# linnil1/KIR_graph

Hardware: AMD Instinct MI355X
Metric: typed 150 bp PE reads/s (pileup+EM) per GPU; achieved HBM GB/s vs roofline (higher is better)
Workload: dtype f64

## Files before the change

include/graphkir_hip.h:

```cpp
#ifndef GRAPHKIR_HIP_H
#define GRAPHKIR_HIP_H

#include <stddef.h>
#include <stdint.h>

#ifdef __cplusplus
extern "C" {
#endif

#define GK_ABI_VERSION 1

#define GK_OK 0
#define GK_ERR_NO_DEVICE (-1)
#define GK_ERR_HIP (-2)
#define GK_ERR_ARG (-3)
#define GK_ERR_ASSERT (-4)
#define GK_ERR_CAPACITY (-5)

#define GK_MAX_CIG 14
#define GK_MAX_MM 16
#define GK_MAX_INS 6
#define GK_MAX_EVENTS 22
#define GK_CIG_M 0
#define GK_CIG_I 1
// ... 132 lines not shown
                       int32_t n_entries, int32_t n_slots, uint64_t* totals_out, int64_t max_out, int32_t* slot_out,
                       int32_t* ord_out, uint32_t* count_out, uint64_t* key_out, int64_t* n_out);

int gk_lut_create(gk_ctx* ctx, int32_t log2_capacity, gk_lut** out);
int gk_lut_destroy(gk_lut* lut);
int gk_lut_collect(gk_lut* lut, gk_dptr d_vals, int64_t n);
int gk_lut_pending(gk_lut* lut, int32_t* n_total, int32_t* n_known);
int gk_lut_export(gk_lut* lut, int32_t first, int32_t count, double* keys_out);
int gk_lut_define(gk_lut* lut, int32_t first, int32_t count, const double* log_vals);
int gk_lut_apply(gk_lut* lut, gk_dptr d_in, gk_dptr d_out, int64_t n);
typedef int (*gk_log10_fn)(const double* values, int64_t n, double* out);
int gk_lut_resolve(gk_lut* lut, gk_log10_fn log10_fn, int32_t* n_new, int32_t* n_known, int32_t* n_undefined);
int gk_lut_resolve_stored(gk_lut* lut, gk_log10_fn log10_fn, int32_t* n_new, int32_t* n_known, int32_t* n_undefined);
int gk_lut_known(gk_lut* lut, int32_t* n_known);
int gk_compat_log(gk_ctx* ctx, gk_tab* tab, gk_dptr d_rows, int64_t n_rows, gk_dptr d_vflag,
                  int32_t vbeg, int32_t vend, gk_dptr d_mask, int32_t words, int32_t n_allele, int32_t keep_empty,
                  gk_lut* lut, gk_dptr d_log);

int gk_maxsum(gk_ctx* ctx, gk_dptr d_L, int64_t n_rows, int64_t ld, const int32_t* ids, int32_t n_sets,
              int32_t c_prev, const int32_t* cols, int32_t n_cols, double* out);
int gk_fraction(gk_ctx* ctx, gk_dptr d_L, int64_t n_rows, int64_t ld, const int32_t* ids,
                int32_t n_sets, int32_t c, double* frac_out);
int gk_setmax(gk_ctx* ctx, gk_dptr d_L, int64_t n_rows, int64_t ld, const int32_t* ids, int32_t n_sets,
              int32_t c, gk_dptr d_P);

int gk_compat_log_miss(gk_ctx* ctx, gk_tab* tab, gk_dptr d_rows, int64_t n_rows, gk_dptr d_vflag,
                       int32_t vbeg, int32_t vend, gk_dptr d_mask, int32_t words, int32_t n_allele,
                       int32_t keep_empty, gk_lut* lut, gk_dptr d_log, gk_dptr d_miss8, int64_t ldm, gk_dptr d_flags);
int gk_miss_colsum(gk_ctx* ctx, gk_dptr d_miss8, int64_t ldm, int32_t n_cols, gk_dptr d_msum);
int gk_compat_log_miss_cols(gk_ctx* ctx, gk_tab* tab, gk_dptr d_rows, int64_t n_rows, gk_dptr d_vflag,
                            int32_t vbeg, int32_t vend, gk_dptr d_mask, int32_t words, int32_t n_allele,
                            int32_t keep_empty, gk_lut* lut, const int32_t* table_cols, int32_t n_table_cols,
                            gk_dptr d_log, gk_dptr d_miss8, int64_t ldm, gk_dptr d_flags);
int gk_compat_patch(gk_ctx* ctx, gk_lut* lut, gk_dptr d_log, int64_t n_rows, int32_t n_allele, gk_dptr d_miss8,
                    int64_t ldm, gk_dptr d_flags);
int gk_compat_index(gk_ctx* ctx, gk_tab* tab, gk_dptr d_rows, int64_t n_rows, gk_dptr d_vflag, int32_t vbeg,
                    int32_t vend, gk_dptr d_mask, int32_t words, int32_t n_allele, int32_t keep_empty, gk_lut* lut,
                    gk_dptr d_lidx, gk_dptr d_miss8, int64_t ldm, gk_dptr d_flags);
int gk_expand_index(gk_ctx* ctx, gk_lut* lut, gk_dptr d_lidx, int64_t ldi, int64_t n_rows, int32_t n_allele, gk_dptr d_L,
                    int64_t ld);
int gk_bound_step(gk_ctx* ctx, gk_dptr d_miss8, int64_t ldm, int64_t n_rows, gk_dptr d_msum, const int32_t* ids,
                  int32_t n_sets, int32_t c_prev, const int32_t* cols, int32_t n_cols, const uint8_t* first,
                  int32_t top_n, int32_t cap, uint32_t* hdr_out, int32_t* idx_out, uint32_t* m_out);
int gk_setsum(gk_ctx* ctx, gk_dptr d_L, int64_t n_rows, int64_t ld, const int32_t* ids, int32_t n_sets, int32_t c,
              double* value_out, double* frac_out);

typedef int (*gk_argsort_fn)(const double* values, int64_t n, int64_t* order_out);
typedef struct gk_search gk_search;
int gk_search_run(gk_ctx* ctx, gk_dptr d_L, int64_t n_rows, int64_t ld, int32_t n_allele, gk_dptr d_miss8,
                  int64_t ldm, gk_dptr d_msum, const int32_t* cols, int32_t n_cols, int32_t n_steps, int32_t top_n,
                  gk_argsort_fn argsort, const double* colsum_in, gk_search** out);
typedef struct gk_gene_job {
  gk_dptr d_rows;
  int64_t n_rows;
  gk_dptr d_mask;
  gk_dptr d_L;
  gk_dptr d_miss8;
  int64_t ldm;
  gk_dptr d_msum;
  gk_dptr d_flags;
  gk_dptr d_lidx;
  int32_t vbeg, vend;
  int32_t words, n_allele;
  int32_t n_steps, top_n;
  int32_t bound_ok, passes;
  int32_t indexed, patches;
// ... 128 lines not shown
```

kir_graph_amd/_lib.py:

```python
from __future__ import annotations

import ctypes as C
import threading
import os
from pathlib import Path

import numpy as np

LIB_NAME = "libgraphkir_hip.so"
_lib = None


class GkError(RuntimeError):
    """Error reported by the native library."""


class GkNoDevice(GkError):
    """No HIP device: the typing path cannot run (there is no CPU fallback)."""


_MM = np.dtype([("ref_off", "<u2"), ("base", "u1"), ("rsv", "u1")])
MATE_DTYPE = np.dtype([
    ("pos0", "<u4"), ("flag", "<u2"), ("ref", "u1"), ("nh", "u1"),
    ("nm", "u1"), ("n_cig", "u1"), ("n_mm", "u1"), ("n_ins", "u1"),
# ... 136 lines not shown
    "gk_bam_next": (C.c_int, [C.c_void_p, C.c_void_p, C.c_int64, C.POINTER(C.c_int64)]),
    "gk_compat_log": (C.c_int, [C.c_void_p, C.c_void_p, C.c_uint64, C.c_int64, C.c_uint64, C.c_int32, C.c_int32,
                                C.c_uint64, C.c_int32, C.c_int32, C.c_int32, C.c_void_p, C.c_uint64]),
    "gk_maxsum": (C.c_int, [C.c_void_p, C.c_uint64, C.c_int64, C.c_int64, C.c_void_p, C.c_int32, C.c_int32,
                            C.c_void_p, C.c_int32, C.c_void_p]),
    "gk_fraction": (C.c_int, [C.c_void_p, C.c_uint64, C.c_int64, C.c_int64, C.c_void_p, C.c_int32, C.c_int32,
                              C.c_void_p]),
    "gk_setmax": (C.c_int, [C.c_void_p, C.c_uint64, C.c_int64, C.c_int64, C.c_void_p, C.c_int32, C.c_int32,
                            C.c_uint64]),
    "gk_packer_create": (C.c_int, [C.c_void_p, C.c_int32, C.c_void_p, C.c_int32, C.POINTER(C.c_void_p)]),
    "gk_packer_destroy": (C.c_int, [C.c_void_p]),
    "gk_packer_feed": (C.c_int, [C.c_void_p, C.c_char_p, C.c_size_t, C.c_int32]),
    "gk_packer_counts": (C.c_int, [C.c_void_p, C.POINTER(C.c_int64), C.POINTER(C.c_int64), C.POINTER(C.c_int64),
                                   C.POINTER(C.c_int64), C.POINTER(C.c_int64)]),
    "gk_packer_error": (C.c_int, [C.c_void_p, C.POINTER(C.c_int32), C.POINTER(C.c_int64)]),
    "gk_packer_records": (C.c_int, [C.c_void_p, C.c_void_p, C.c_void_p]),
    "gk_packer_set_output": (C.c_int, [C.c_void_p, C.c_void_p, C.c_int64]),
    "gk_packer_spilled": (C.c_int, [C.c_void_p, C.POINTER(C.c_int64)]),
    "gk_packer_spill_records": (C.c_int, [C.c_void_p, C.c_void_p, C.c_void_p]),
    "gk_packer_string": (C.c_char_p, [C.c_void_p, C.c_int64]),
    "gk_depth": (C.c_int, [C.c_void_p, C.c_void_p, C.c_uint64, C.c_int32, C.c_void_p, C.c_int32, C.c_void_p]),
    "gk_depth_write_tsv": (C.c_int, [C.c_char_p, C.c_void_p, C.c_void_p, C.c_int32, C.c_void_p]),
    "gk_cn_fit": (C.c_int, [C.c_void_p, C.c_void_p, C.c_void_p, C.c_int32, C.c_void_p, C.c_int32, C.c_void_p,
                            C.c_int32, C.c_int32, C.c_double, C.c_void_p]),
    "gk_cn_assign": (C.c_int, [C.c_void_p, C.c_void_p, C.c_int32, C.c_double, C.c_void_p, C.c_int32, C.c_int32,
                               C.c_double, C.c_void_p]),
    "gk_em_sets": (C.c_int, [C.c_void_p, C.c_void_p, C.c_uint64, C.c_int64, C.c_int32, C.c_int32, C.c_uint64,
                             C.c_int32, C.c_uint64]),
    "gk_em_distinct": (C.c_int, [C.c_void_p, C.c_uint64, C.c_int64, C.c_int32, C.c_int32, C.c_void_p, C.c_void_p,
                                 C.POINTER(C.c_int32)]),
    "gk_compat_log_miss_cols": (C.c_int, [C.c_void_p, C.c_void_p, C.c_uint64, C.c_int64, C.c_uint64, C.c_int32, C.c_int32,
                                          C.c_uint64, C.c_int32, C.c_int32, C.c_int32, C.c_void_p, C.c_void_p, C.c_int32,
                                          C.c_uint64, C.c_uint64, C.c_int64, C.c_uint64]),
    "gk_compat_log_miss": (C.c_int, [C.c_void_p, C.c_void_p, C.c_uint64, C.c_int64, C.c_uint64, C.c_int32, C.c_int32,
                                     C.c_uint64, C.c_int32, C.c_int32, C.c_int32, C.c_void_p, C.c_uint64, C.c_uint64,
                                     C.c_int64, C.c_uint64]),
    "gk_miss_colsum": (C.c_int, [C.c_void_p, C.c_uint64, C.c_int64, C.c_int32, C.c_uint64]),
    "gk_compat_index": (C.c_int, [C.c_void_p, C.c_void_p, C.c_uint64, C.c_int64, C.c_uint64, C.c_int32, C.c_int32,
                                  C.c_uint64, C.c_int32, C.c_int32, C.c_int32, C.c_void_p, C.c_uint64, C.c_uint64,
                                  C.c_int64, C.c_uint64]),
    "gk_expand_index": (C.c_int, [C.c_void_p, C.c_void_p, C.c_uint64, C.c_int64, C.c_int64, C.c_int32, C.c_uint64,
                                  C.c_int64]),
    "gk_bound_step": (C.c_int, [C.c_void_p, C.c_uint64, C.c_int64, C.c_int64, C.c_uint64, C.c_void_p, C.c_int32,
                                C.c_int32, C.c_void_p, C.c_int32, C.c_void_p, C.c_int32, C.c_int32, C.c_void_p,
                                C.c_void_p, C.c_void_p]),
    "gk_setsum": (C.c_int, [C.c_void_p, C.c_uint64, C.c_int64, C.c_int64, C.c_void_p, C.c_int32, C.c_int32,
                            C.c_void_p, C.c_void_p]),
    "gk_search_run": (C.c_int, [C.c_void_p, C.c_uint64, C.c_int64, C.c_int64, C.c_int32, C.c_uint64, C.c_int64,
                                C.c_uint64, C.c_void_p, C.c_int32, C.c_int32, C.c_int32, C.c_void_p, C.c_void_p,
                                C.POINTER(C.c_void_p)]),
    "gk_sample_search": (C.c_int, [C.c_void_p, C.c_void_p, C.c_int32, C.c_void_p, C.c_uint64, C.c_void_p, C.c_void_p,
                                   C.c_int32, C.c_void_p, C.c_void_p, C.c_void_p]),
    "gk_lut_resolve": (C.c_int, [C.c_void_p, C.c_void_p, C.POINTER(C.c_int32), C.POINTER(C.c_int32),
                                 C.POINTER(C.c_int32)]),
    "gk_sample_prepare_exon": (C.c_int, [C.c_void_p, C.c_void_p, C.c_int32, C.c_uint64, C.c_uint64, C.c_uint64, C.c_void_p,
                                         C.c_int64, C.c_void_p, C.c_void_p, C.c_void_p, C.POINTER(C.c_int64)]),
    "gk_sample_em": (C.c_int, [C.c_void_p, C.c_void_p, C.c_void_p, C.c_int32, C.c_int32, C.c_double, C.c_void_p, C.c_void_p]),
    "gk_mates_compact": (C.c_int, [C.c_void_p, C.c_uint64, C.c_int64, C.POINTER(C.c_uint64), C.POINTER(C.c_int64)]),
    "gk_mates_expand": (C.c_int, [C.c_void_p, C.c_uint64, C.c_int64, C.c_uint64]),
    "gk_mates_compact_size": (C.c_int, [C.c_void_p, C.c_int64, C.c_int32, C.POINTER(C.c_int64)]),
    "gk_mates_compact_host": (C.c_int, [C.c_void_p, C.c_int64, C.c_int32, C.c_void_p, C.c_int64]),
    "gk_compat_patch": (C.c_int, [C.c_void_p, C.c_void_p, C.c_uint64, C.c_int64, C.c_int32, C.c_uint64, C.c_int64, C.c_uint64]),
    "gk_lut_resolve_stored": (C.c_int, [C.c_void_p, C.c_void_p, C.POINTER(C.c_int32), C.POINTER(C.c_int32),
                                        C.POINTER(C.c_int32)]),
    "gk_lut_known": (C.c_int, [C.c_void_p, C.POINTER(C.c_int32)]),
    "gk_search_steps": (C.c_int, [C.c_void_p, C.POINTER(C.c_int32)]),
# ... 288 lines not shown
```

kir_graph_amd/build.py:

```python
from __future__ import annotations

import os
import shutil
import subprocess
from pathlib import Path

PKG = Path(__file__).resolve().parent
ROOT = PKG.parent
SOURCES = ["gk_runtime.hip", "gk_scan.hip", "gk_tabulate.hip", "gk_typing.hip", "gk_lut.hip",
           "gk_search.hip", "gk_bound.hip", "gk_em.hip", "gk_cn.hip", "gk_depth.hip", "gk_sampack.cpp", "gk_bamread.cpp", "gk_textout.cpp",
           "gk_comm.cpp", "gk_hostsearch.cpp", "gk_novel.hip", "gk_boot.hip"]


def hipcc() -> str:
    for cand in (os.environ.get("HIPCC"), shutil.which("hipcc"), "/opt/rocm/bin/hipcc"):
        if cand and Path(cand).exists():
            return cand
    raise RuntimeError("hipcc not found (set HIPCC)")


def outOfDate(lib: Path) -> bool:
    if not lib.exists():
        return True
    t = lib.stat().st_mtime
    deps = [PKG / "csrc" / s for s in SOURCES] + list((PKG / "csrc").glob("*.h")) + [ROOT / "include" / "graphkir_hip.h"]
    return any(d.stat().st_mtime > t for d in deps)


KERNEL_SOURCES = {
    "compat_kernel": ["gk_typing.hip", "gk_lut.h", "gk_common.h"],
    "patch_pending": ["gk_typing.hip", "gk_lut.h", "gk_common.h"],
    "count_ids_genes": ["gk_typing.hip", "gk_common.h"],
    "flag_nonempty": ["gk_typing.hip", "gk_common.h"],
    "flag_pairs": ["gk_typing.hip", "gk_common.h"],
    "gather_pair_flags": ["gk_typing.hip", "gk_common.h"],
    "tab_count": ["gk_tabulate.hip", "gk_common.h"],
    "tab_emit": ["gk_tabulate.hip", "gk_common.h"],
    "tab_expand": ["gk_tabulate.hip", "gk_common.h"],
    "minsum_sad": ["gk_bound.hip", "gk_common.h"],
    "minsum_finish": ["gk_bound.hip", "gk_common.h"],
    "select_hist1": ["gk_bound.hip", "gk_common.h"],
    "select_hist2": ["gk_bound.hip", "gk_common.h"],
    "select_append": ["gk_bound.hip", "gk_common.h"],
    "setmin_u8": ["gk_bound.hip", "gk_common.h"],
    "fraction_chunks": ["gk_search.hip", "gk_common.h"],
    "setsum_leaves": ["gk_search.hip", "gk_common.h"],
    "fold_leaves": ["gk_search.hip", "gk_common.h"],
    "colsum_chunks": ["gk_search.hip", "gk_common.h"],
    "maxsum_chunks": ["gk_search.hip", "gk_common.h"],
    "combine_chunks": ["gk_search.hip", "gk_common.h"],
    "em_sets_groups": ["gk_em.hip", "gk_common.h"],
    "em_sets_hash": ["gk_em.hip", "gk_common.h"],
    "em_sets_verify": ["gk_em.hip", "gk_common.h"],
    "em_sets_emit": ["gk_em.hip", "gk_common.h"],
    "em_kernel_genes": ["gk_em.hip", "gk_squarem.h", "gk_common.h"],
    "novel_assign": ["gk_novel.hip", "gk_common.h"],
    "novel_confusion": ["gk_novel.hip", "gk_common.h"],
    "novel_compact": ["gk_novel.hip", "gk_common.h"],
    "boot_resample": ["gk_boot.hip", "gk_common.h"],
    "boot_em_batch": ["gk_boot.hip", "gk_squarem.h", "gk_common.h"],
}


# ... 51 lines not shown
```

kir_graph_amd/csrc/gk_hostsearch.cpp:

```cpp
#include <algorithm>
#include <cmath>
#include <memory>
#include <numeric>
#include <string>
#include <unordered_map>
#include <unordered_set>
#include <chrono>
#include <sys/syscall.h>
#include <unistd.h>

#include "gk_calls.h"
#include "gk_lut.h"

namespace {

struct Step {
  int n = 0;
  int bounded = 0;
  std::vector<double> value, sum_indv, frac;
  std::vector<int32_t> ids;
  int64_t rows() const { return (int64_t)value.size(); }
};

inline double sum_small(const double* a, int n) {
// ... 139 lines not shown
    for (size_t i = 0; i < n; ++i)
      if (!seen[ids[i]]) { seen[ids[i]] = 1; ++d; }
    return d;
  }
  void note(int64_t kind, int64_t a, int64_t b, int64_t c, int64_t d, int64_t e, int64_t f) {
    const int64_t row[7] = {kind, a, b, c, d, e, f};
    log.insert(log.end(), row, row + 7);
  }
  void to_alleles(const int32_t* cols, int n_cols, int n_alleles) {
    for (Step& st : steps)
      for (int32_t& id : st.ids) id = cols[id];
    table_cols.assign(cols, cols + n_cols);
    n_full = n_alleles;
  }
};

extern "C" {

int gk_maxsum(gk_ctx* ctx, gk_dptr d_L, int64_t n_rows, int64_t ld, const int32_t* ids, int32_t n_sets, int32_t c_prev,
              const int32_t* cols, int32_t n_cols, double* out);
int gk_fraction(gk_ctx* ctx, gk_dptr d_L, int64_t n_rows, int64_t ld, const int32_t* ids, int32_t n_sets, int32_t c,
                double* frac_out);
int gk_compat_log_miss(gk_ctx* ctx, gk_tab* tab, gk_dptr d_rows, int64_t n_rows, gk_dptr d_vflag, int32_t vbeg,
                       int32_t vend, gk_dptr d_mask, int32_t words, int32_t n_allele, int32_t keep_empty, gk_lut* lut,
                       gk_dptr d_log, gk_dptr d_miss8, int64_t ldm, gk_dptr d_flags);
int gk_compat_log(gk_ctx* ctx, gk_tab* tab, gk_dptr d_rows, int64_t n_rows, gk_dptr d_vflag, int32_t vbeg,
                  int32_t vend, gk_dptr d_mask, int32_t words, int32_t n_allele, int32_t keep_empty, gk_lut* lut,
                  gk_dptr d_log);
__attribute__((weak)) int gk_compat_log_miss_cols(gk_ctx* ctx, gk_tab* tab, gk_dptr d_rows, int64_t n_rows, gk_dptr d_vflag,
                                                  int32_t vbeg, int32_t vend, gk_dptr d_mask, int32_t words, int32_t n_allele,
                                                  int32_t keep_empty, gk_lut* lut, const int32_t* table_cols,
                                                  int32_t n_table_cols, gk_dptr d_log, gk_dptr d_miss8, int64_t ldm,
                                                  gk_dptr d_flags);
int gk_miss_colsum(gk_ctx* ctx, gk_dptr d_miss8, int64_t ldm, int32_t n_cols, gk_dptr d_msum);
int gk_compat_patch(gk_ctx* ctx, gk_lut* lut, gk_dptr d_log, int64_t n_rows, int32_t n_allele, gk_dptr d_miss8, int64_t ldm,
                    gk_dptr d_flags);
int gk_compat_index(gk_ctx* ctx, gk_tab* tab, gk_dptr d_rows, int64_t n_rows, gk_dptr d_vflag, int32_t vbeg, int32_t vend,
                    gk_dptr d_mask, int32_t words, int32_t n_allele, int32_t keep_empty, gk_lut* lut, gk_dptr d_lidx,
                    gk_dptr d_miss8, int64_t ldm, gk_dptr d_flags);

}

namespace {

struct GeneSearch {
  gk_ctx* ctx = nullptr;
  GkTable table;
  gk_dptr d_L = 0;
  void* expanded = nullptr;
  gk_dptr d_miss8 = 0, d_msum = 0;
  int64_t n_rows = 0, ld = 0, ldm = 0;
  int n_allele = 0, n_steps = 0, T = 0, A = 0;
  std::vector<int32_t> cols;
  std::vector<std::vector<int32_t>> step_cols;
  gk_argsort_fn argsort = nullptr;
  bool bound = false, unique_cols = true;
  std::unique_ptr<gk_search> S;
  std::vector<uint8_t> first;
  int64_t N = 0;
  GkBoundCall bcall;
  GkSumCall scall;
  Head sel;
  Step st;
  bool bound_in_flight = false, sums_in_flight = false, step_done = false;

  int init(gk_ctx* c, const GkTable& tbl, gk_dptr L, int64_t rows, int64_t ld_, int32_t n_allele_, gk_dptr miss8, int64_t ldm_,
// ... 547 lines not shown
  std::vector<std::unique_ptr<GeneSearch>> gs((size_t)n_jobs);
  enum { kTable, kBound, kSums, kOneSet };
  struct Item { int gene, stage; uint64_t mark; };
  std::deque<Item> queue;
  struct OneSetBatch { GkSumCall call; std::vector<int> deps; int k = 0; std::vector<int32_t> ids; };
  std::vector<std::unique_ptr<OneSetBatch>> batches;
  auto fail = [&](int code) {
    gk_fetch_cancel(ctx);
    for (auto& g : gs) if (g) g->abandon();
    for (auto& b : batches) if (b) gk_release(ctx, b->call.temps);
    return code;
  };
  auto push = [&](int gene, int stage) {
    uint64_t m = 0;
    const int r = set_mark(ctx, &m);
    if (r == GK_OK) queue.push_back({gene, stage, m});
    return r;
  };
  std::vector<uint32_t> sticky((size_t)n_jobs, 0);
  auto n_cols_of = [&](int i) { return jobs[i].n_table_cols > 0 ? jobs[i].n_table_cols : jobs[i].n_allele; };
  auto col_of = [&](int owner, int32_t a, int32_t* col) -> int {
    const gk_gene_job& o = jobs[owner];
    if (a < 0 || a >= o.n_allele) { gk_set_error("candidate allele out of range"); return GK_ERR_ARG; }
    if (o.n_table_cols <= 0) { *col = a; return GK_OK; }
    const int32_t* const end = o.table_cols + o.n_table_cols;
    const int32_t* const at = std::lower_bound(o.table_cols, end, a);
    if (at == end || *at != a) {
      gk_set_error("candidate allele %d is not among the columns of its table", (int)a);
      return GK_ERR_ARG;
    }
    *col = (int32_t)(at - o.table_cols);
    return GK_OK;
  };
  auto write_table = [&](int i, bool patch) -> int {
    gk_gene_job& j = jobs[i];
    const int nc = n_cols_of(i);
    int rc;
    if (patch) {
      j.patches++;
      sticky[i] |= flags[i] & 1u;
      rc = gk_compat_patch(ctx, lut, j.d_L, j.n_rows, nc, j.d_miss8, j.ldm, j.d_flags);
    } else {
      j.passes++;
      sticky[i] = 0;
      if (j.n_table_cols > 0)
        rc = gk_compat_log_miss_cols(ctx, tab, j.d_rows, j.n_rows, d_vflag, j.vbeg, j.vend, j.d_mask, j.words, j.n_allele, 0,
                                     lut, j.table_cols, j.n_table_cols, j.d_L, j.d_miss8, j.ldm, j.d_flags);
      else
        rc = gk_compat_log_miss(ctx, tab, j.d_rows, j.n_rows, d_vflag, j.vbeg, j.vend, j.d_mask, j.words, j.n_allele, 0, lut,
                                j.d_L, j.d_miss8, j.ldm, j.d_flags);
    }
    if (rc == GK_OK) rc = gk_miss_colsum(ctx, j.d_miss8, j.ldm, nc, j.d_msum);
    if (rc == GK_OK && gk_fetch_queue(ctx, &flags[i], gk_ptr<void>(j.d_flags), sizeof(uint32_t)) != hipSuccess) rc = GK_ERR_HIP;
    if (rc) return rc;
    std::vector<int32_t> cols((size_t)nc);
    std::iota(cols.begin(), cols.end(), 0);
    if (gs[i]) gs[i]->abandon();
    gs[i].reset(new GeneSearch());
    rc = gs[i]->init(ctx, GkTable{j.d_L, j.n_rows, nullptr}, j.d_L, j.n_rows, j.n_rows, nc, j.d_miss8, j.ldm, j.d_msum,
                     cols.data(), nc, j.n_steps, j.top_n, argsort);
    if (rc == GK_OK) rc = gs[i]->colsum_enqueue();
    if (rc == GK_OK) rc = push(i, kTable);
    return rc;
  };
  std::vector<std::vector<int>> dependents((size_t)n_jobs);
  for (int i : live)
    if (jobs[i].table_of >= 0) dependents[(size_t)jobs[i].table_of].push_back(i);
  int rc = GK_OK;
  for (int i : live) {
    if (jobs[i].table_of >= 0) continue;
    rc = write_table(i, false);
    if (rc) return fail(rc);
  }

  auto advance = [&](int i, bool at_step_start) -> int {
    GeneSearch& g = *gs[i];
    for (;;) {
      if (at_step_start) {
// ... 379 lines not shown
```

kir_graph_amd/roofmodel.py:

```python
from __future__ import annotations

HBM_PEAK_GBS = 8000.0
TILE = 32
N_SIMD = 256 * 4
NOMINAL_HZ = 2.4e9

ISSUE_CYCLES = {"v_mul_f64": 4.50, "v_add_f64": 4.26, "v_max_f64": 4.19, "v_bfe_i32": 4.43, "v_bfi_b32": 4.56,
                "v_sad_u8": 4.49}
GUIDE_CYCLES = {"v_mul_f64": 4.0, "v_add_f64": 4.0, "v_max_f64": 4.0, "v_bfe_i32": 2.0, "v_bfi_b32": 2.0, "v_sad_u8": 2.0}
SEQUENCE_CYCLES = {"compat_kernel": 5.81}
KERNEL_OPS = {
    "compat_kernel": ("v_bfe_i32", "v_bfi_b32", "v_bfi_b32", "v_mul_f64"),
    "minsum_sad": ("v_sad_u8",),
    "maxsum_chunks": ("v_max_f64", "v_add_f64"),
}


def laneOpsPeak(kernel: str, table: dict[str, float] = ISSUE_CYCLES) -> float:
    ops = KERNEL_OPS[kernel]
    return len(ops) * 64 * N_SIMD * NOMINAL_HZ / sum(table[o] for o in ops)


def symmetricOutputs(n: int) -> int:
    total = 0
    for t0 in range(0, n, TILE):
        rows = min(TILE, n - t0)
        total += rows * (n - t0)
    return total


def maxsumLaunch(n_rows: int, n_sets: int, c_prev: int, n_cols: int, n_prev_cols: int,
                 symmetric: bool = False) -> tuple[float, float]:
    by = 8.0 * n_rows * (n_cols + n_prev_cols) + 8.0 * n_sets * n_cols
    outputs = symmetricOutputs(n_cols) if symmetric else n_sets * n_cols
    return by, 2.0 * n_rows * outputs


def minsumLaunch(n_rows: int, n_sets: int, n_cols: int, n_prev_cols: int, symmetric: bool = False
                 ) -> tuple[float, float]:
    outputs = symmetricOutputs(n_cols) if symmetric else n_sets * n_cols
    return 1.0 * n_rows * (n_cols + n_prev_cols) + 4.0 * n_sets * n_cols, n_rows * outputs / 4.0


def compatLaunch(n_rows: int, n_allele: int, n_ids: float, out_bytes: int = 8) -> tuple[float, float]:
    return 4.0 * n_ids + 16.0 * n_rows + float(out_bytes + 1) * n_rows * n_allele, 4.0 * n_ids * n_allele
# ... 1 lines not shown

def tabLaunch(n_pairs: int, n_valid: int, n_ids: int) -> tuple[float, float]:
    return 256.0 * n_pairs + 4.0 * n_ids + 22.0 * n_valid, 0.0


def setsumLaunch(n_rows: int, n_sets: int, c: int, n_distinct: int) -> tuple[float, float]:
    return 8.0 * n_rows * n_distinct + 8.0 * n_sets * (c + 1), float(n_rows) * n_sets * (c + 1)


def emSetsLaunch(n_rows: int, n_ids: float, set_words: int) -> tuple[float, float]:
    return 24.0 * n_rows + 4.0 * n_ids + 4.0 * set_words, 0.0


def emVerifyLaunch(set_words: int) -> tuple[float, float]:
    return 4.0 * set_words, 0.0


def _priced(kernel: str, calls: list[tuple]) -> tuple[float, float, str, float]:
    by = ops = 0.0
    bound, peak = "hbm", 0.0
    for c in calls:
        if kernel == "maxsum_chunks":
            b, o = maxsumLaunch(*c[1:7])
            bound, peak = "valu", laneOpsPeak("maxsum_chunks")
        elif kernel == "colsum_chunks":
            b, o = 8.0 * c[1] * c[4] + 8.0 * c[4], 0.0
        elif kernel == "em_sets_groups":
            b, o = emSetsLaunch(*c[1:4])
        elif kernel == "em_sets_verify":
            b, o = emVerifyLaunch(c[3])
        elif kernel == "minsum_sad":
            b, o = minsumLaunch(*c[1:6])
            bound, peak = "valu", laneOpsPeak("minsum_sad")
        elif kernel == "compat_kernel":
            b, o = compatLaunch(*c[1:5])
            bound, peak = "valu", laneOpsPeak("compat_kernel")
        elif kernel == "tab_count":
            b, o = tabLaunch(*c[1:4])
        elif kernel in ("fraction_chunks", "setsum_leaves"):
            b, o = setsumLaunch(*c[1:5])
        else:
            return 0.0, 0.0, "hbm", 0.0
        by += b
        ops += o
    return by, ops, bound, peak


def summarise(call_log: list[tuple], kernel: str, total_ms: float, launches: int) -> dict:
    calls = [c for c in call_log if c[0] == kernel]
    base = {"kernel": kernel, "bound": "hbm", "achieved": None, "peak": HBM_PEAK_GBS, "unit": "GB/s",
            "frac": None, "traffic": None, "launches": launches, "avg_launch_ms": total_ms / max(launches, 1)}
    if not calls or total_ms <= 0:
        return base
    by, ops, bound, peak = _priced(kernel, calls)
    if by <= 0:
        return base
    sec = total_ms / 1e3
    gbs = by / sec / 1e9
    hbm = {"achieved": gbs, "peak": HBM_PEAK_GBS, "unit": "GB/s", "frac": gbs / HBM_PEAK_GBS}
    out = dict(base)
    out["algorithmic_bytes_per_launch"] = by / max(launches, 1)
    if bound == "valu":
        tops = ops / sec / 1e12
        unit = {"maxsum_chunks": "Tops/s f64 (max+add)", "minsum_sad": "T lane-ops/s (v_sad_u8, 4 reads each)",
                "compat_kernel": "T lane-ops/s (4 VALU per id and allele)"}.get(kernel, "T lane-ops/s")
        guide = laneOpsPeak(kernel, GUIDE_CYCLES)
        out.update({"bound": "valu", "achieved": tops, "peak": peak / 1e12, "unit": unit, "frac": ops / sec / peak,
                    "peak_guide": guide / 1e12, "frac_guide": ops / sec / guide,
                    "issue_cycles": {o: ISSUE_CYCLES[o] for o in KERNEL_OPS[kernel]},
                    "algorithmic_ops_per_launch": ops / max(launches, 1), "hbm": hbm,
                    "note": "VALU-issue bound (ordered f64 products / a (max,+) or (min,+) contraction).  `peak` = the "
                            "kernel's own instruction mix issued back to back at the MEASURED cost of each instruction "
                            "(tools/valu_rate.hip at 8 waves per SIMD, profiles/r03_valu_rate.txt: cycles of a 2.4 GHz "
                            "clock per wave64 instruction and SIMD in `issue_cycles`); `peak_guide` / `frac_guide` price "
                            "the same mix at the guide's 2 cycles per 32-bit and 4 per float64 instruction.  The HBM "
                            "roof is shown beside it; symmetric launches are credited with the triangle of tiles they "
                            "compute"})
        if kernel in SEQUENCE_CYCLES:
            seq = 64 * N_SIMD * NOMINAL_HZ / SEQUENCE_CYCLES[kernel]
            out["peak_sequence"] = seq / 1e12
            out["frac_sequence"] = ops / sec / seq
            out["note"] += (".  `peak_sequence` / `frac_sequence`: the same instructions at the rate measured for them "
                            "as the sequence the kernel issues (eight independent chains per wave, 8 waves per SIMD)")
    else:
        out.update(hbm)
        out["bound"] = "hbm"
    return out


def dominant(prof: dict[str, tuple[int, float]], call_log: list[tuple]) -> dict:
    if not prof:
        return summarise([], "none", 0.0, 0)
    priced = {k: v for k, v in prof.items() if _priced(k, [c for c in call_log if c[0] == k])[0] > 0}
    top = max(prof.items(), key=lambda kv: kv[1][1])[0]
    name, (launches, total_ms) = max((priced or prof).items(), key=lambda kv: kv[1][1])
    out = summarise(call_log, name, total_ms, launches)
    total = sum(v[1] for v in prof.values())
    out["share_of_kernel_time"] = total_ms / total if total else None
# ... 42 lines not shown
```

kir_graph_amd/typing_mulit_allele.py:

```python
from __future__ import annotations

from collections import defaultdict
from dataclasses import dataclass, field
from itertools import chain
from typing import Iterable, Optional

import threading

import numpy as np

from ._lib import Device, DeviceBuffer
from .engine import DeviceModel, LogTable, PreparedGene, Tabulation
from .index import buildMask
from .msa2hisat import Variant
from .utils import logger

SEARCH_STATS = {"bounded": 0, "redone_exactly": 0}
_default_logs: dict[int, LogTable] = {}
_default_logs_lock = threading.Lock()


def nativeSearch() -> bool:
    return True


_GROUP_CACHE_LOCK = threading.Lock()


def sharedLogTable(dev: Device) -> LogTable:
    with _default_logs_lock:
        t = _default_logs.get(dev.ordinal)
        if t is None:
            t = _default_logs[dev.ordinal] = LogTable(dev, private_context=True)
    return t


@dataclass
class TypingResult:

    n: int
    value: np.ndarray
    value_sum_indv: np.ndarray
    allele_id: np.ndarray
    allele_name: list[list[str]]
    allele_prob: "np.ndarray | LazyAlleleProb"
    fraction: np.ndarray
    fraction_uniq: np.ndarray
    allele_name_group: list[list[list[str]]] = field(default_factory=list)

    def isFail(self) -> bool:
        return not len(self.value)

    def selectBest(self, filter_fraction: bool = True, filter_minor: bool = False) -> list[str]:
        ids: Iterable[int] = range(len(self.fraction))
        if filter_fraction and len(self.fraction):
            floor = (1 / self.n) / 2
            ids = np.flatnonzero((np.asarray(self.fraction) >= floor).all(axis=1)).tolist()
        if filter_minor:
            ids = [i for i in ids
                   if np.abs(self.value_sum_indv[i]).min() / np.abs(self.value_sum_indv[i]).max() > 0.8]
        best = (list(ids) or [0])[0]
        if not self.isFail():
            logger.debug(f"[Allele] Select best rank: {best}")
            assert len(self.allele_name[best]) == self.n
            return self.allele_name[best]
        logger.warning("[Allele] No candidates found. Return fail")
        return ["fail"] * self.n
# ... 523 lines not shown
            elif kind == 1:
                m.dev.call_log.append(("minsum_sad", a, b, c_, d, False))
            else:
                m.dev.call_log.append(("setsum_leaves" if kind == 3 else "fraction_chunks", a, b, c_, d))

    def geneJob(self, cn: int, verdict: bool | None = None):
        from ._lib import GeneJob
        if cn < 1:
            raise ValueError(f"CN should be >= 1, got {cn}")
        if self.force_homo is not None:
            homo = self.force_homo
        else:
            homo = self._isHomozygous(cn) if verdict is None else verdict
        m = self._model
        vbeg, vend, mask, words = m._geom
        cols = m._table_cols
        job = GeneJob(d_rows=m.rows.ptr, n_rows=m.n_rows, d_mask=mask.ptr, d_L=m._L.ptr if m._L else 0,
                      d_miss8=m.miss8.ptr if m.miss8 else 0, ldm=m.ldm, d_msum=m.msum.ptr if m.msum else 0,
                      d_flags=m._bound_flags.ptr if m._bound_flags else 0, d_lidx=m.lidx.ptr if m.lidx else 0,
                      vbeg=vbeg, vend=vend, words=words, n_allele=m.n_allele, n_steps=1 if homo else cn,
                      top_n=self.top_n, bound_ok=0, passes=0, indexed=0, patches=0, table_of=-1, n_step_cols=0,
                      step_cols=None, step_cols_off=None, table_cols=None if cols is None else cols.ctypes.data,
                      n_table_cols=0 if cols is None else len(cols))
        return job, homo

    def adoptJob(self, job, handle, cn: int, homo: bool) -> TypingResult:
        m = self._model
        m._bound_ok = bool(job.bound_ok)
        m._indexed = bool(job.indexed)
        m._known_at_launch = -1
        if m.dev.call_log is not None:
            per_row = m.tab.n_ids / max(m.tab.n_valid, 1)
            for _ in range(max(1, int(job.passes))):
                m.dev.call_log.append(("compat_kernel", m.n_rows, m.n_allele, per_row * m.n_rows, 2 if m._indexed else 8))
        self.result = []
        self._adoptSearch(handle, 1 if homo else cn)
        if homo:
            self.addHomoResultForCn(cn)
        self.result[-1].print()
        return self.result[-1]

    def adoptTable(self, job, handle) -> None:
        import ctypes as C
        from ._lib import check, lib
        m = self._model
        m._bound_ok = bool(job.bound_ok)
        m._indexed = False
        m._known_at_launch = -1
        n_written = m.n_allele if m._table_cols is None else len(m._table_cols)
        if m.dev.call_log is not None:
            per_row = m.tab.n_ids / max(m.tab.n_valid, 1)
            for _ in range(max(1, int(job.passes))):
                m.dev.call_log.append(("compat_kernel", m.n_rows, n_written, per_row * m.n_rows, 8))
            self._logLaunches(handle)
        colsum = np.empty(m.n_allele, dtype=np.float64)
        check(lib().gk_search_colsum(handle, colsum.ctypes.data))
        self._colsum_all = colsum if m._table_cols is None else None
        self.result = []

    def addHomoResultForCn(self, cn: int) -> None:
        if cn > 1:
            self.result.append(self.createHomoResult(self.result[0], cn))

    @staticmethod
    def createHomoResult(cn1_result: TypingResult, cn: int) -> TypingResult:
        if cn <= 1:
            raise ValueError(f"CN should be > 1, got {cn}")
        if cn1_result.isFail():
            e = np.array([])
            return TypingResult(cn, e, e, e, [], e, e, e)
        m = len(cn1_result.value)
        return TypingResult(
            n=cn, value=cn1_result.value * cn,
            value_sum_indv=np.repeat(cn1_result.value_sum_indv, cn, axis=1),
            allele_id=np.repeat(cn1_result.allele_id, cn, axis=1),
            allele_name=[[row[0]] * cn for row in cn1_result.allele_name],
            allele_prob=cn1_result.allele_prob,
            fraction=np.ones((m, cn)) / cn, fraction_uniq=np.ones((m, cn)) / cn)

    @staticmethod
    def uniqueAllele(data: np.ndarray) -> np.ndarray:
        return firstOccurrence(np.asarray(data), int(np.max(data)) + 1 if np.size(data) else 1)

    def _colsums(self) -> np.ndarray:
        if self._colsum_all is None:
            self.finish()
# ... 462 lines not shown
```

Measured before the change: 427.9 million.

## Add specialized narrow compatibility kernel for tables with at most eight columns

Adds a dedicated kernel for compatibility tables of up to 8 columns. A pre-pass packs the selected mask bits into one byte per variant. The main kernel then has each wave handle 8 rows, with 8 lanes per row, one lane per column. Ids are compacted through ballot into LDS strips so the log-probability products use byte-packed bits instead of reading the wide mask for every allele. The host search dispatches to this path when the column count is 1–8. This adds an extra launch, a pool allocation per table, and tile-to-XCD scheduling logic.

```diff
diff --git a/include/graphkir_hip.h b/include/graphkir_hip.h
--- a/include/graphkir_hip.h
+++ b/include/graphkir_hip.h
@@ -188,6 +188,10 @@
                             int32_t vbeg, int32_t vend, gk_dptr d_mask, int32_t words, int32_t n_allele,
                             int32_t keep_empty, gk_lut* lut, const int32_t* table_cols, int32_t n_table_cols,
                             gk_dptr d_log, gk_dptr d_miss8, int64_t ldm, gk_dptr d_flags);
+int gk_compat_log_miss_narrow(gk_ctx* ctx, gk_tab* tab, gk_dptr d_rows, int64_t n_rows, gk_dptr d_vflag,
+                              int32_t vbeg, int32_t vend, gk_dptr d_mask, int32_t words, int32_t n_allele,
+                              int32_t keep_empty, gk_lut* lut, const int32_t* table_cols, int32_t n_table_cols,
+                              gk_dptr d_log, gk_dptr d_miss8, int64_t ldm, gk_dptr d_flags);
 int gk_compat_patch(gk_ctx* ctx, gk_lut* lut, gk_dptr d_log, int64_t n_rows, int32_t n_allele, gk_dptr d_miss8,
                     int64_t ldm, gk_dptr d_flags);
 int gk_compat_index(gk_ctx* ctx, gk_tab* tab, gk_dptr d_rows, int64_t n_rows, gk_dptr d_vflag, int32_t vbeg,
diff --git a/kir_graph_amd/_lib.py b/kir_graph_amd/_lib.py
--- a/kir_graph_amd/_lib.py
+++ b/kir_graph_amd/_lib.py
@@ -192,6 +192,9 @@
     "gk_compat_log_miss_cols": (C.c_int, [C.c_void_p, C.c_void_p, C.c_uint64, C.c_int64, C.c_uint64, C.c_int32, C.c_int32,
                                           C.c_uint64, C.c_int32, C.c_int32, C.c_int32, C.c_void_p, C.c_void_p, C.c_int32,
                                           C.c_uint64, C.c_uint64, C.c_int64, C.c_uint64]),
+    "gk_compat_log_miss_narrow": (C.c_int, [C.c_void_p, C.c_void_p, C.c_uint64, C.c_int64, C.c_uint64, C.c_int32, C.c_int32,
+                                            C.c_uint64, C.c_int32, C.c_int32, C.c_int32, C.c_void_p, C.c_void_p, C.c_int32,
+                                            C.c_uint64, C.c_uint64, C.c_int64, C.c_uint64]),
     "gk_compat_log_miss": (C.c_int, [C.c_void_p, C.c_void_p, C.c_uint64, C.c_int64, C.c_uint64, C.c_int32, C.c_int32,
                                      C.c_uint64, C.c_int32, C.c_int32, C.c_int32, C.c_void_p, C.c_uint64, C.c_uint64,
                                      C.c_int64, C.c_uint64]),
diff --git a/kir_graph_amd/build.py b/kir_graph_amd/build.py
--- a/kir_graph_amd/build.py
+++ b/kir_graph_amd/build.py
@@ -9,7 +9,7 @@
 ROOT = PKG.parent
 SOURCES = ["gk_runtime.hip", "gk_scan.hip", "gk_tabulate.hip", "gk_typing.hip", "gk_lut.hip",
            "gk_search.hip", "gk_bound.hip", "gk_em.hip", "gk_cn.hip", "gk_depth.hip", "gk_sampack.cpp", "gk_bamread.cpp", "gk_textout.cpp",
-           "gk_comm.cpp", "gk_hostsearch.cpp", "gk_novel.hip", "gk_boot.hip"]
+           "gk_comm.cpp", "gk_hostsearch.cpp", "gk_novel.hip", "gk_boot.hip", "gk_compat_narrow.hip"]
 
 
 def hipcc() -> str:
@@ -29,6 +29,7 @@
 
 KERNEL_SOURCES = {
     "compat_kernel": ["gk_typing.hip", "gk_lut.h", "gk_common.h"],
+    "compat_narrow": ["gk_compat_narrow.hip", "gk_lut.h", "gk_common.h"],
     "patch_pending": ["gk_typing.hip", "gk_lut.h", "gk_common.h"],
     "count_ids_genes": ["gk_typing.hip", "gk_common.h"],
     "flag_nonempty": ["gk_typing.hip", "gk_common.h"],
diff --git a/kir_graph_amd/csrc/gk_compat_narrow.hip b/kir_graph_amd/csrc/gk_compat_narrow.hip
--- /dev/null
+++ b/kir_graph_amd/csrc/gk_compat_narrow.hip
@@ -0,0 +1,224 @@
+#include <algorithm>
+
+#include "gk_common.h"
+#include "gk_lut.h"
+
+namespace {
+
+constexpr int kThreads = 256;
+constexpr int kMaxCols = 8;
+constexpr int kWaveRows = 8;
+constexpr int kWaves = 8;
+constexpr int kNarrowThreads = 64 * kWaves;
+constexpr int kTileRows = kWaveRows * kWaves;
+constexpr int kStripWords = 17;
+
+struct NarrowCols { int32_t a[kMaxCols]; };
+
+__global__ __launch_bounds__(kThreads) void narrow_bits(const uint32_t* __restrict__ mask, int n_span, int words,
+                                                        NarrowCols cols, int n_cols, uint8_t* __restrict__ out,
+                                                        uint32_t* zero_word) {
+  if (blockIdx.x == 0 && threadIdx.x == 0) *zero_word = 0;
+  const int v = blockIdx.x * kThreads + threadIdx.x;
+  if (v >= n_span) return;
+  const uint32_t* const row = mask + (int64_t)v * words;
+  uint32_t x = 0;
+#pragma unroll
+  for (int c = 0; c < kMaxCols; ++c) {
+    const int a = cols.a[c];
+    if (c < n_cols) x |= ((row[a >> 5] >> (a & 31)) & 1u) << c;
+  }
+  out[v] = (uint8_t)x;
+}
+
+__global__ __launch_bounds__(kNarrowThreads) void compat_narrow(const int32_t* __restrict__ rows, int64_t n_rows,
+                                                                const uint32_t* __restrict__ off,
+                                                                const uint32_t* __restrict__ ids,
+                                                                const uint8_t* __restrict__ vflag, int vbeg, int n_span,
+                                                                const uint8_t* __restrict__ bits8, int n_cols,
+                                                                double* __restrict__ logs, LutView lut, double empty_p,
+                                                                uint8_t* __restrict__ miss8, int64_t ldm,
+                                                                uint32_t* flags) {
+  __shared__ uint32_t strips[kWaves][kWaveRows][kStripWords];
+  constexpr int32_t kHi999 = 0x3FEFF7CE, kLo999 = (int32_t)0xD916872B, kHi001 = 0x3F50624D, kLo001 = (int32_t)0xD2F1A9FC;
+  const int tid = threadIdx.x, lane = tid & 63;
+  const int wid = __builtin_amdgcn_readfirstlane(tid >> 6);
+  const int r = lane >> 3, c = lane & 7;
+  const int64_t n_tiles = (n_rows + kTileRows - 1) / kTileRows;
+  const int64_t n_groups = (n_tiles + 1) / 2;
+  const int xcd = blockIdx.x & 7;
+  const int64_t my_groups = n_groups > xcd ? (n_groups - xcd + 7) / 8 : 0;
+  const int64_t wg_per_xcd = gridDim.x >> 3;
+  for (int64_t u = blockIdx.x >> 3; u < 2 * my_groups; u += wg_per_xcd) {
+    const int64_t tile_i = 2 * (xcd + 8 * (u >> 1)) + (u & 1);
+    if (tile_i >= n_tiles) continue;
+    const int64_t row0 = tile_i * kTileRows + wid * kWaveRows;
+    uint32_t my_b, my_mid, my_e;
+    {
+      const int64_t i = row0 + c;
+      const int64_t row = rows[i < n_rows ? i : n_rows - 1];
+      my_b = off[4 * row]; my_mid = off[4 * row + 2]; my_e = off[4 * row + 4];
+      if (i >= n_rows) my_b = my_mid = my_e;
+    }
+    uint32_t b[kWaveRows], mid[kWaveRows], e[kWaveRows];
+    uint32_t longest = 0;
+#pragma unroll
+    for (int q = 0; q < kWaveRows; ++q) {
+      b[q] = (uint32_t)__builtin_amdgcn_readlane((int)my_b, q);
+      mid[q] = (uint32_t)__builtin_amdgcn_readlane((int)my_mid, q);
+      e[q] = (uint32_t)__builtin_amdgcn_readlane((int)my_e, q);
+      longest = max(longest, e[q] > b[q] ? e[q] - b[q] : 0u);
+    }
+    double p = 1.0;
+    uint32_t n_var = 0;
+    uint8_t* const wave_bytes = reinterpret_cast<uint8_t*>(&strips[wid][0][0]);
+    const uint32_t* const my_strip = &strips[wid][r][0];
+    for (uint32_t done = 0; done < longest; done += 64) {
+      uint32_t k[kWaveRows], v[kWaveRows], x[kWaveRows];
+      uint8_t dropped[kWaveRows];
+#pragma unroll
+      for (int q = 0; q < kWaveRows; ++q) {
+        k[q] = b[q] + done + (uint32_t)lane;
+        v[q] = ids[k[q] < e[q] ? k[q] : (e[q] ? e[q] - 1u : 0u)];
+      }
+#pragma unroll
+      for (int q = 0; q < kWaveRows; ++q) {
+        const uint32_t local = v[q] - (uint32_t)vbeg;
+        const bool indexed = local < (uint32_t)n_span;
+        dropped[q] = vflag[v[q]];
+        const uint32_t got = bits8[indexed ? local : 0u];
+        x[q] = indexed ? got : 0u;
+      }
+      uint32_t my_count = 0, most = 0, least = 64;
+#pragma unroll
+      for (int q = 0; q < kWaveRows; ++q) {
+        const bool positive = k[q] < mid[q];
+        const bool keep = k[q] < e[q] && !(dropped[q] & (positive ? 1 : 2));
+        const uint64_t kept = __ballot(keep);
+        const uint32_t n_kept = (uint32_t)__builtin_popcountll(kept);
+        const uint32_t place =
+            __builtin_amdgcn_mbcnt_hi((uint32_t)(kept >> 32), __builtin_amdgcn_mbcnt_lo((uint32_t)kept, 0u));
+        wave_bytes[4 * kStripWords * q + (keep ? place : 64u)] = (uint8_t)(positive ? x[q] : ~x[q]);
+        my_count = r == q ? n_kept : my_count;
+        most = max(most, n_kept);
+        least = min(least, n_kept);
+      }
+      __builtin_amdgcn_wave_barrier();
+      auto factor = [&](uint32_t w, int j) {
+        const int32_t m = __builtin_amdgcn_sbfe((int32_t)w, 8 * j + c, 1);
+        return __hiloint2double((m & kHi999) | (~m & kHi001), (m & kLo999) | (~m & kLo001));
+      };
+      const uint32_t all = least & ~3u;
+#pragma unroll 2
+      for (uint32_t t = 0; t < all; t += 4) {
+        const uint32_t w = my_strip[t >> 2];
+#pragma unroll
+        for (int j = 0; j < 4; ++j) p *= factor(w, j);
+      }
+      for (uint32_t t = all; t < most; t += 4) {
+        const uint32_t w = my_strip[t >> 2];
+        const int left = (int)my_count - (int)t;
+#pragma unroll
+        for (int j = 0; j < 4; ++j) {
+          const double f = factor(w, j);
+          p *= j < left ? f : 1.0;
+        }
+      }
+      __builtin_amdgcn_wave_barrier();
+      n_var += my_count;
+    }
+    const int64_t i = row0 + r;
+    const bool mine = i < n_rows && c < n_cols;
+    uint32_t raise = 0;
+    if (mine && n_var >= 4096u) raise |= 1u;
+    uint32_t m8 = 0;
+    if (mine) {
+      const double prod = n_var ? p : empty_p;
+      const uint64_t key = (uint64_t)__double_as_longlong(prod);
+      bool found;
+      double val = gk_lut_lookup(lut, key, &found);
+      if (!found) {
+        gk_lut_insert(lut, key);
+        const bool marks = (int64_t)key > 0;
+        raise |= marks ? 4u : 12u;
+        if (marks) val = prod;
+      }
+      logs[(int64_t)c * n_rows + i] = val;
+      const double t = __builtin_fma(val, -1.0 / 3.0, 0.25);
+      if (t < 100.0) m8 = (uint32_t)(int)t;
+      else { m8 = 255u; if (val == val) raise |= 1u; }
+    }
+    {
+      uint32_t packed = m8;
+      packed |= (uint32_t)__shfl_down((int)m8, 8, 64) << 8;
+      packed |= (uint32_t)__shfl_down((int)m8, 16, 64) << 16;
+      packed |= (uint32_t)__shfl_down((int)m8, 24, 64) << 24;
+      if ((r & 3) == 0 && c < n_cols) *reinterpret_cast<uint32_t*>(miss8 + (int64_t)c * ldm + i) = packed;
+    }
+    {
+      const uint32_t bits = (__ballot((raise & 1u) != 0) ? 1u : 0u) | (__ballot((raise & 4u) != 0) ? 4u : 0u) |
+                            (__ballot((raise & 8u) != 0) ? 8u : 0u);
+      if (bits && lane == 0) atomicOr(flags, bits);
+    }
+    if (tile_i == n_tiles - 1) {
+      const int64_t pad0 = n_tiles * kTileRows;
+      const int n_pad = (int)((ldm - pad0) / 4);
+      for (int it = tid; it < n_cols * n_pad; it += kNarrowThreads) {
+        const int al = it / n_pad, w = it % n_pad;
+        *reinterpret_cast<uint32_t*>(miss8 + (int64_t)al * ldm + pad0 + 4 * w) = 0u;
+      }
+    }
+  }
+}
+
+}
+
+extern "C" {
+
+int gk_compat_log_miss_narrow(gk_ctx* ctx, gk_tab* tab, gk_dptr d_rows, int64_t n_rows, gk_dptr d_vflag, int32_t vbeg,
+                              int32_t vend, gk_dptr d_mask, int32_t words, int32_t n_allele, int32_t keep_empty,
+                              gk_lut* lut, const int32_t* table_cols, int32_t n_table_cols, gk_dptr d_log,
+                              gk_dptr d_miss8, int64_t ldm, gk_dptr d_flags) {
+  gk_bind(ctx);
+  GK_REQUIRE(ctx && tab && lut, "null pointer");
+  GK_REQUIRE(words >= 1 && n_allele >= 0 && n_allele <= words * 32 && vend >= vbeg, "bad mask geometry");
+  NarrowCols cols{};
+  int n_cols;
+  if (table_cols) {
+    GK_REQUIRE(n_table_cols >= 1 && n_table_cols <= n_allele, "bad column list");
+    GK_REQUIRE(n_table_cols <= kMaxCols, "a narrow compatibility table has at most 8 columns");
+    for (int c = 0; c < n_table_cols; ++c) {
+      GK_REQUIRE(table_cols[c] >= 0 && table_cols[c] < n_allele && (c == 0 || table_cols[c] > table_cols[c - 1]),
+                 "table columns must be allele ordinals, ascending and unique");
+      cols.a[c] = table_cols[c];
+    }
+    n_cols = n_table_cols;
+  } else {
+    GK_REQUIRE(n_table_cols == 0, "a column count without a column list");
+    GK_REQUIRE(n_allele <= kMaxCols, "a narrow compatibility table has at most 8 columns");
+    for (int c = 0; c < n_allele; ++c) cols.a[c] = c;
+    n_cols = n_allele;
+  }
+  if (n_rows == 0 || n_cols == 0) return GK_OK;
+  GK_REQUIRE(n_rows > 0 && d_log && d_miss8 && d_flags, "null output");
+  GK_REQUIRE(ldm >= n_rows && ldm % 64 == 0, "mismatch table stride must be a multiple of 64 rows");
+  const int n_span = vend - vbeg;
+  uint8_t* bits8 = nullptr;
+  if (gk_pool_malloc(ctx, (void**)&bits8, (size_t)std::max(n_span, 1)) != hipSuccess) {
+    gk_set_error("out of device memory for the columns' bits");
+    return GK_ERR_HIP;
+  }
+  GK_KERNEL(narrow_bits, dim3((unsigned)std::max(1, (n_span + kThreads - 1) / kThreads)), dim3(kThreads), 0, ctx->stream,
+            gk_ptr<uint32_t>(d_mask), n_span, words, cols, n_cols, bits8, gk_ptr<uint32_t>(d_flags));
+  const int64_t want = ((n_rows + kTileRows - 1) / kTileRows + 7) / 8 * 8;
+  const dim3 grid((unsigned)(want < 2048 ? want : 2048)), block(kNarrowThreads);
+  GK_PROF(ctx, "compat_narrow",
+          GK_KERNEL(compat_narrow, grid, block, 0, ctx->stream, gk_ptr<int32_t>(d_rows), n_rows, tab->d_off, tab->d_ids,
+                    gk_ptr<uint8_t>(d_vflag), vbeg, n_span, bits8, n_cols, gk_ptr<double>(d_log), gk_lut_view(lut),
+                    keep_empty ? 0.999 : 1.0, gk_ptr<uint8_t>(d_miss8), ldm, gk_ptr<uint32_t>(d_flags)));
+  gk_pool_free(ctx, bits8);
+  GK_HIP(hipGetLastError());
+  return GK_OK;
+}
+
+}
diff --git a/kir_graph_amd/csrc/gk_hostsearch.cpp b/kir_graph_amd/csrc/gk_hostsearch.cpp
--- a/kir_graph_amd/csrc/gk_hostsearch.cpp
+++ b/kir_graph_amd/csrc/gk_hostsearch.cpp
@@ -195,6 +195,11 @@
                                                   int32_t keep_empty, gk_lut* lut, const int32_t* table_cols,
                                                   int32_t n_table_cols, gk_dptr d_log, gk_dptr d_miss8, int64_t ldm,
                                                   gk_dptr d_flags);
+__attribute__((weak)) int gk_compat_log_miss_narrow(gk_ctx* ctx, gk_tab* tab, gk_dptr d_rows, int64_t n_rows, gk_dptr d_vflag,
+                                                    int32_t vbeg, int32_t vend, gk_dptr d_mask, int32_t words,
+                                                    int32_t n_allele, int32_t keep_empty, gk_lut* lut,
+                                                    const int32_t* table_cols, int32_t n_table_cols, gk_dptr d_log,
+                                                    gk_dptr d_miss8, int64_t ldm, gk_dptr d_flags);
 int gk_miss_colsum(gk_ctx* ctx, gk_dptr d_miss8, int64_t ldm, int32_t n_cols, gk_dptr d_msum);
 int gk_compat_patch(gk_ctx* ctx, gk_lut* lut, gk_dptr d_log, int64_t n_rows, int32_t n_allele, gk_dptr d_miss8, int64_t ldm,
                     gk_dptr d_flags);
@@ -808,6 +813,7 @@
     *col = (int32_t)(at - o.table_cols);
     return GK_OK;
   };
+  const bool narrow = gk_compat_log_miss_narrow && !gk_test_hook("wide_tables");
   auto write_table = [&](int i, bool patch) -> int {
     gk_gene_job& j = jobs[i];
     const int nc = n_cols_of(i);
@@ -819,7 +825,11 @@
     } else {
       j.passes++;
       sticky[i] = 0;
-      if (j.n_table_cols > 0)
+      if (narrow && nc >= 1 && nc <= 8)
+        rc = gk_compat_log_miss_narrow(ctx, tab, j.d_rows, j.n_rows, d_vflag, j.vbeg, j.vend, j.d_mask, j.words, j.n_allele, 0,
+                                       lut, j.n_table_cols > 0 ? j.table_cols : nullptr, j.n_table_cols, j.d_L, j.d_miss8,
+                                       j.ldm, j.d_flags);
+      else if (j.n_table_cols > 0)
         rc = gk_compat_log_miss_cols(ctx, tab, j.d_rows, j.n_rows, d_vflag, j.vbeg, j.vend, j.d_mask, j.words, j.n_allele, 0,
                                      lut, j.table_cols, j.n_table_cols, j.d_L, j.d_miss8, j.ldm, j.d_flags);
       else
diff --git a/kir_graph_amd/roofmodel.py b/kir_graph_amd/roofmodel.py
--- a/kir_graph_amd/roofmodel.py
+++ b/kir_graph_amd/roofmodel.py
@@ -8,9 +8,10 @@
 ISSUE_CYCLES = {"v_mul_f64": 4.50, "v_add_f64": 4.26, "v_max_f64": 4.19, "v_bfe_i32": 4.43, "v_bfi_b32": 4.56,
                 "v_sad_u8": 4.49}
 GUIDE_CYCLES = {"v_mul_f64": 4.0, "v_add_f64": 4.0, "v_max_f64": 4.0, "v_bfe_i32": 2.0, "v_bfi_b32": 2.0, "v_sad_u8": 2.0}
-SEQUENCE_CYCLES = {"compat_kernel": 5.81}
+SEQUENCE_CYCLES = {"compat_kernel": 5.81, "compat_narrow": 5.81}
 KERNEL_OPS = {
     "compat_kernel": ("v_bfe_i32", "v_bfi_b32", "v_bfi_b32", "v_mul_f64"),
+    "compat_narrow": ("v_bfe_i32", "v_bfi_b32", "v_bfi_b32", "v_mul_f64"),
     "minsum_sad": ("v_sad_u8",),
     "maxsum_chunks": ("v_max_f64", "v_add_f64"),
 }
@@ -78,9 +79,9 @@
         elif kernel == "minsum_sad":
             b, o = minsumLaunch(*c[1:6])
             bound, peak = "valu", laneOpsPeak("minsum_sad")
-        elif kernel == "compat_kernel":
+        elif kernel in ("compat_kernel", "compat_narrow"):
             b, o = compatLaunch(*c[1:5])
-            bound, peak = "valu", laneOpsPeak("compat_kernel")
+            bound, peak = "valu", laneOpsPeak(kernel)
         elif kernel == "tab_count":
             b, o = tabLaunch(*c[1:4])
         elif kernel in ("fraction_chunks", "setsum_leaves"):
@@ -109,7 +110,8 @@
     if bound == "valu":
         tops = ops / sec / 1e12
         unit = {"maxsum_chunks": "Tops/s f64 (max+add)", "minsum_sad": "T lane-ops/s (v_sad_u8, 4 reads each)",
-                "compat_kernel": "T lane-ops/s (4 VALU per id and allele)"}.get(kernel, "T lane-ops/s")
+                "compat_kernel": "T lane-ops/s (4 VALU per id and allele)",
+                "compat_narrow": "T lane-ops/s (4 VALU per id and column)"}.get(kernel, "T lane-ops/s")
         guide = laneOpsPeak(kernel, GUIDE_CYCLES)
         out.update({"bound": "valu", "achieved": tops, "peak": peak / 1e12, "unit": unit, "frac": ops / sec / peak,
                     "peak_guide": guide / 1e12, "frac_guide": ops / sec / guide,
diff --git a/kir_graph_amd/typing_mulit_allele.py b/kir_graph_amd/typing_mulit_allele.py
--- a/kir_graph_amd/typing_mulit_allele.py
+++ b/kir_graph_amd/typing_mulit_allele.py
@@ -33,6 +33,12 @@
         if t is None:
             t = _default_logs[dev.ordinal] = LogTable(dev, private_context=True)
     return t
+
+
+def _tableKernel(n_cols: int, indexed: bool = False) -> str:
+    from .utils import testHook
+    narrow = 1 <= n_cols <= 8 and not indexed and testHook("wide_tables") is None
+    return "compat_narrow" if narrow else "compat_kernel"
 
 
 @dataclass
@@ -622,7 +628,8 @@
         if m.dev.call_log is not None:
             per_row = m.tab.n_ids / max(m.tab.n_valid, 1)
             for _ in range(max(1, int(job.passes))):
-                m.dev.call_log.append(("compat_kernel", m.n_rows, m.n_allele, per_row * m.n_rows, 2 if m._indexed else 8))
+                m.dev.call_log.append((_tableKernel(m.n_allele, m._indexed), m.n_rows, m.n_allele, per_row * m.n_rows,
+                                       2 if m._indexed else 8))
         self.result = []
         self._adoptSearch(handle, 1 if homo else cn)
         if homo:
@@ -641,7 +648,7 @@
         if m.dev.call_log is not None:
             per_row = m.tab.n_ids / max(m.tab.n_valid, 1)
             for _ in range(max(1, int(job.passes))):
-                m.dev.call_log.append(("compat_kernel", m.n_rows, n_written, per_row * m.n_rows, 8))
+                m.dev.call_log.append((_tableKernel(n_written), m.n_rows, n_written, per_row * m.n_rows, 8))
             self._logLaunches(handle)
         colsum = np.empty(m.n_allele, dtype=np.float64)
         check(lib().gk_search_colsum(handle, colsum.ctypes.data))
```

Result: slower. 410.1 million (-4.2%).
